# AI4Science-WestlakeU/wdno

Hardware: AMD Instinct MI355X
Metric: diffusion train steps/sec, 2D smoke U-Net (8 samples per GPU per step) (higher is better)
Workload: dtype f32

## Files before the change

### include/wdno_hip.h

```cpp
#ifndef WDNO_HIP_H
#define WDNO_HIP_H
#include <stdint.h>
#include <stddef.h>

#ifdef __cplusplus
extern "C" {
#endif

typedef void* wdno_stream_t;

enum { WDNO_OK = 0, WDNO_EINVAL = -1, WDNO_ELAUNCH = -2, WDNO_EUNSUPPORTED = -3, WDNO_EWORKSPACE = -4 };

#define WDNO_AMAX_SLOTS 64
#define WDNO_AMAX_STRIDE 16
#define WDNO_AMAX_FLOATS (WDNO_AMAX_SLOTS * WDNO_AMAX_STRIDE)
const char* wdno_strerror(int code);
int wdno_version(void);
const char* wdno_last_hip_error(void);
int wdno_set_debug(int mode);

typedef struct {
  int nd;
  int mode;
  int L;
  int n_img;
  int in_dims[3];
  int out_dims[3];
  int64_t cs_img, cs_band, cs0, cs1;
} wdno_dwt_desc;
size_t wdno_dwt_ws_bytes(const wdno_dwt_desc* d);
int wdno_dwt_fwd(const float* x, float* coef, const wdno_dwt_desc* d, const float* filters_host, void* ws, size_t ws_bytes, wdno_stream_t s);
int wdno_dwt_inv(const float* coef, float* x, const wdno_dwt_desc* d, const float* filters_host, void* ws, size_t ws_bytes, wdno_stream_t s);
int wdno_dwt_fwd_adjoint(const float* dcoef, float* dx, const wdno_dwt_desc* d, const float* filters_host, void* ws, size_t ws_bytes, wdno_stream_t s);
int wdno_dwt_inv_adjoint(const float* dx, float* dcoef, const wdno_dwt_desc* d, const float* filters_host, void* ws, size_t ws_bytes, wdno_stream_t s);
int wdno_dwt_fwd_packed(const float* x, float* state, const wdno_dwt_desc* d, const float* filters_host, int img_inner, int64_t cs_outer, int row_w,
                        const float* rescaler, wdno_stream_t s);
int wdno_upsample_coef(const float* in, float* out, int64_t outer, int a, int mid, int b, int c, int fa, int fb, int fc, wdno_stream_t s);
int wdno_pack_smoke_state(const float* coef, int64_t coef_sim_stride, const float* init_coef, int64_t init_sim_stride, const float* smokeout,
                          int64_t so_sim_stride, const int64_t* idx, const float* rescaler, float* state, int64_t B, int F, int nt, int nx,
                          int pad_t, int pad_x, wdno_stream_t s);
int wdno_pack_smoke_fields(const float* coef, int64_t coef_sim_stride, const float* rho0, int64_t rho0_sim_stride, const float* curve,
                           int64_t curve_sim_stride, const float* dec_lo_host, const float* dec_hi_host, int L, const float* rescaler,
                           float* state, int64_t B, int F, int nt, int nx, int pad_t, int pad_x, int H0, int W0, int T0, wdno_stream_t s);

int wdno_nc_to_cl(const float* src, float* dst, int64_t N, int C, int64_t S, int Cp, wdno_stream_t s);
int wdno_cl_to_nc(const float* src, float* dst, int64_t N, int C, int64_t S, int Cp, wdno_stream_t s);
int wdno_concat2_cl_planes(const float* a, int Ca, const float* b, int Cb, const float* rec_a, const float* rec_b, void* hi, void* lo,
                           float* scale_out, int64_t P, wdno_stream_t s);
int wdno_concat2_cl(const float* a, int Ca, const float* b, int Cb, float* out, int64_t P, wdno_stream_t s);
int wdno_concat2_cl_amax(const float* a, int Ca, const float* b, int Cb, float* out, float* amax_rec, int64_t P, wdno_stream_t s);
int wdno_split2_cl(const float* in, float* a, int Ca, float* b, int Cb, int64_t P, wdno_stream_t s);
int wdno_upsample2x_cl_fwd(const float* in, float* out, int64_t N, int H, int W, int C, wdno_stream_t s);
int wdno_upsample2x_cl_bwd(const float* dout, float* din, int64_t N, int H, int W, int C, wdno_stream_t s);

typedef struct {
  int N, D, H, W, C;
  int OD, OH, OW, K;
  int kd, kh, kw;
  int sd, sh, sw;
  int pd, ph, pw;
  int YD, YH, YW;
  int osd, osh, osw, ood, ooh, oow;
} wdno_conv_geom;
int wdno_conv_fwd(const float* x, const float* wp, const float* bias, const float* residual, float* y,
                  const wdno_conv_geom* g, wdno_stream_t s);
int wdno_amax(const float* x, int64_t n, float* amax_zeroed, wdno_stream_t s);
int wdno_amax_record(const float* x, int64_t n, float* rec_zeroed, wdno_stream_t s);
int wdno_split_f16(const float* x, const float* amax_rec, void* hi, void* lo, float* scale_out, int64_t rows, int C, int C8, wdno_stream_t s);
size_t wdno_split_colsum_ws_bytes(int64_t rows, int C8);
int wdno_split_f16_colsum(const float* x, const float* amax_rec, void* hi, void* lo, float* scale_out, float* colsum_out,
                          void* ws, size_t ws_bytes, int64_t rows, int C, int C8, wdno_stream_t s);
int wdno_pack_split_weight(const float* w, const float* amax, void* hi, void* lo, float* scale_out, int K, int C, int kd, int kh, int kw,
                           int A, int B, int mode, wdno_stream_t s);
typedef struct { const void* x; int64_t n; void* out; } wdno_amax_item;
typedef struct {
  const void* w; const void* amax; void* hi; void* lo; void* scale_out;
  int K, C, kd, kh, kw, A, B, mode;
} wdno_wsplit_item;
int wdno_amax_multi(const void* table, int n_items, int blocks_per_item, wdno_stream_t s);
int wdno_pack_split_weight_multi(const void* table, int n_items, int blocks_per_item, wdno_stream_t s);
int wdno_conv_fwd_f16x3(const void* xh, const void* xl, const float* sx, const void* wph, const void* wpl, const float* sw,
                        const float* bias, const float* residual, float* y, const wdno_conv_geom* g, wdno_stream_t s);
int wdno_conv_fwd_f16x3_amax(const void* xh, const void* xl, const float* sx, const void* wph, const void* wpl, const float* sw,
                             const float* bias, const float* residual, float* y, float* amax_rec, const wdno_conv_geom* g,
                             wdno_stream_t s);
typedef struct { int channels, d0, h0, w0; } wdno_zero_box;
int wdno_conv_fwd_f16x3_zbox(const void* xh, const void* xl, const float* sx, const void* wph, const void* wpl, const float* sw,
                             const float* bias, const float* residual, float* y, float* amax_rec, const wdno_conv_geom* g,
                             const wdno_zero_box* zb, wdno_stream_t s);
int wdno_conv_fwd_bf16_ex(const void* x16, const void* wp16, const float* bias, const float* residual, void* y, int y_bf16, float* amax_rec,
                          const wdno_conv_geom* g, const wdno_zero_box* zb, wdno_stream_t s);
int wdno_conv_fwd_f16x3_ws(const void* xh, const void* xl, const float* sx, const void* wph, const void* wpl, const float* sw,
                           const float* bias, const float* residual, float* y, float* amax_rec, const wdno_conv_geom* g,
                           void* ws, size_t ws_bytes, wdno_stream_t s);
size_t wdno_conv_fwd_split_ws_bytes(const wdno_conv_geom* g);
size_t wdno_conv_wgrad_f16x3_ws_bytes(const wdno_conv_geom* g);
int wdno_conv_pixel_table(void* table, const wdno_conv_geom* g, wdno_stream_t s);
int wdno_conv_wgrad_f16x3(const void* xh, const void* xl, const float* sx, const void* dyh, const void* dyl, const float* sdy,
                          const void* pixel_table, float* dwp, void* ws, size_t ws_bytes, const wdno_conv_geom* g, wdno_stream_t s);
int wdno_conv_wgrad_f16x3_param(const void* xh, const void* xl, const float* sx, const void* dyh, const void* dyl, const float* sdy,
                                const void* pixel_table, float* dw, int Kn, int Cn, void* ws, size_t ws_bytes,
                                const wdno_conv_geom* g, wdno_stream_t s);
#define WDNO_WGRAD_REDUCE_MAX 40
typedef struct wdno_wgrad_reduce_item {
  const float* ws; float* dw;
  int n, splits;
  int K8, C8, kw, ntap, Kn, Cn;
  int tiled;
  int reserved;
} wdno_wgrad_reduce_item;
int wdno_conv_wgrad_partials(const void* xh, const void* xl, const float* sx, const void* dyh, const void* dyl, const float* sdy,
                             const void* pixel_table, float* dw, int Kn, int Cn, void* ws, size_t ws_bytes,
                             const wdno_conv_geom* g, wdno_wgrad_reduce_item* item, wdno_stream_t s);
int wdno_wgrad_reduce_multi(const wdno_wgrad_reduce_item* items, int n_items, wdno_stream_t s);
size_t wdno_conv_wgrad_ws_bytes(const wdno_conv_geom* g);
int wdno_conv_wgrad(const float* x, const float* dy, float* dwp, void* ws, size_t ws_bytes,
                    const wdno_conv_geom* g, wdno_stream_t s);
#define WDNO_ROWS_SUM_MAX 64
typedef struct wdno_rows_sum_item {
  const void* part; float* out;
  int rows, stride, col0, ncols;
  int is_double, reserved;
} wdno_rows_sum_item;
int wdno_rows_sum_multi(const wdno_rows_sum_item* items, int n_items, wdno_stream_t s);
size_t wdno_colsum_ws_bytes(int64_t P, int C);
int wdno_colsum(const float* in, float* out, int64_t P, int C, void* ws, size_t ws_bytes, wdno_stream_t s);

int wdno_cast_bf16(const float* x, void* out16, int64_t rows, int C, int C8, wdno_stream_t s);
int wdno_cast_bf16_colsum(const float* x, void* out16, float* colsum_out, void* ws, size_t ws_bytes, int64_t rows, int C, int C8, wdno_stream_t s);
int wdno_conv_fwd_bf16(const void* x16, const void* wp16, const float* bias, const float* residual, float* y, float* amax_rec,
                       const wdno_conv_geom* g, wdno_stream_t s);
int wdno_conv_wgrad_bf16_param(const void* x16, const void* dy16, const void* pixel_table, float* dw, int Kn, int Cn, void* ws,
                               size_t ws_bytes, const wdno_conv_geom* g, wdno_stream_t s);

size_t wdno_groupnorm_ws_bytes(int64_t N, int64_t S, int C, int G);
size_t wdno_groupnorm_stats_floats(int64_t N, int C, int G);
int wdno_groupnorm_act_fwd(const float* x, const float* gamma, const float* beta, const float* ss, float* y,
                           float* stats, int64_t N, int64_t S, int C, int G, float eps, int silu,
                           void* ws, size_t ws_bytes, wdno_stream_t s);
int wdno_groupnorm_act_fwd_amax(const float* x, const float* gamma, const float* beta, const float* ss, float* y,
                                float* stats, float* amax_rec, int64_t N, int64_t S, int C, int G, float eps, int silu,
                                void* ws, size_t ws_bytes, wdno_stream_t s);
int wdno_groupnorm_act_bwd(const float* x, const float* dy, const float* gamma, const float* beta, const float* ss,
                           const float* stats, float* dx, float* dgb_partial, float* dss,
                           int64_t N, int64_t S, int C, int G, int silu, void* ws, size_t ws_bytes, wdno_stream_t s);
int wdno_groupnorm_act_bwd_amax(const float* x, const float* dy, const float* gamma, const float* beta, const float* ss,
                                const float* stats, float* dx, float* dgb_partial, float* dss, float* amax_rec,
                                int64_t N, int64_t S, int C, int G, int silu, void* ws, size_t ws_bytes, wdno_stream_t s);
size_t wdno_groupnorm_bwd_planes_ws_bytes(int64_t N, int64_t S, int C, int G);
size_t wdno_groupnorm_fwd_planes_ws_bytes(int64_t N, int64_t S, int C, int G);
int wdno_groupnorm_act_fwd_planes(const float* x, const float* gamma, const float* beta, const float* ss, void* y_hi, void* y_lo,
                                  float* y_scale, float* stats, float* bound_rec, int64_t N, int64_t S, int C, int G, float eps, int silu,
                                  void* ws, size_t ws_bytes, wdno_stream_t s);
int wdno_groupnorm_act_add_fwd_planes(const float* x, const float* gamma, const float* beta, const float* ss, const float* residual,
                                      const float* res_rec, float* y, void* y_hi, void* y_lo, float* y_scale, float* stats,
                                      float* bound_rec, float* y_amax_rec, int64_t N, int64_t S, int C, int G, float eps, int silu,
                                      void* ws, size_t ws_bytes, wdno_stream_t s);
int wdno_groupnorm_act_bwd_planes(const float* x, const float* dy, const float* gamma, const float* beta, const float* ss,
                                  const float* stats, void* dx_hi, void* dx_lo, float* dx_scale, float* dx_colsum,
                                  float* dgb_partial, float* dgb_sum, float* dss, float* bound_rec, int64_t N, int64_t S, int C, int G, int silu,
                                  void* ws, size_t ws_bytes, wdno_stream_t s);
int wdno_groupnorm_bwd_planes_tail(int64_t N, int64_t S, int C, int G, size_t* csp_offset, int* rows);
int wdno_groupnorm_act_fwd_amax_t(const void* x, int x_bf16, const float* gamma, const float* beta, const float* ss, float* y,
// ... 224 lines not shown
```

### wdno_amd/_lib.py

```python
import contextlib
import ctypes as C
import os

import torch

HERE = os.path.dirname(os.path.abspath(__file__))
LIB_PATH = os.path.join(HERE, 'libwdno_hip.so')

P = C.c_void_p
I = C.c_int
L = C.c_int64
F = C.c_float
Z = C.c_size_t


class DwtDesc(C.Structure):
    _fields_ = [('nd', I), ('mode', I), ('L', I), ('n_img', I), ('in_dims', I * 3), ('out_dims', I * 3),
                ('cs_img', L), ('cs_band', L), ('cs0', L), ('cs1', L)]


class ConvGeom(C.Structure):
    _fields_ = [(k, I) for k in ('N', 'D', 'H', 'W', 'C', 'OD', 'OH', 'OW', 'K', 'kd', 'kh', 'kw', 'sd', 'sh', 'sw',
                                 'pd', 'ph', 'pw', 'YD', 'YH', 'YW', 'osd', 'osh', 'osw', 'ood', 'ooh', 'oow')]


class AttnDesc(C.Structure):
    _fields_ = [('n_uo', I), ('n_ui', I), ('n_tok', I), ('heads', I), ('so', L), ('si', L), ('st', L)]


class CondDesc(C.Structure):
    _fields_ = [(k, I) for k in ('tree', 'B', 'F', 'C', 'H', 'W', 'cT', 'cH', 'cW', 'cond_pad', 'cond_a', 'cond_b',
                                 'cond_c', 'cond_low', 'u_rows', 'uT_rows')]


class WgradReduceItem(C.Structure):
    _fields_ = [('ws', C.c_void_p), ('dw', C.c_void_p), ('n', I), ('splits', I), ('K8', I), ('C8', I), ('kw', I), ('ntap', I), ('Kn', I), ('Cn', I),
                ('tiled', I), ('reserved', I)]


class RowsSumItem(C.Structure):
    _fields_ = [('part', C.c_void_p), ('out', C.c_void_p), ('rows', I), ('stride', I), ('col0', I), ('ncols', I), ('is_double', I), ('reserved', I)]


class BurgersDesc(C.Structure):
    _fields_ = [(k, I) for k in ('N', 's', 'nx0', 'nt_f', 'nxf', 'steps', 'record_time', 'f_time', 'num_t', 'sub_s', 'out_cols', 'waves',
                                 'points')] + [(k, F) for k in ('c', 'd', 'dm', 'dt')]


class BurgersGenerateDesc(C.Structure):
    _fields_ = [(k, I) for k in ('N', 's', 't', 'steps', 'record_time', 'f_time', 'num_t', 'st', 'sx', 'f_rows', 'cols', 'waves', 'points',
                                 'clamp')] + [(k, F) for k in ('c', 'd', 'dm', 'dt', 'alpha')]


class BurgersGuidanceDesc(C.Structure):
    _fields_ = [(k, I) for k in ('B', 'C', 'H', 'W', 'sample_stride', 'chan_stride', 'row_stride', 'h', 'w', 'n_t', 'n_x', 'L', 'mode', 'ntile',
                                 'tw', 'lds_bytes', 'num_timesteps', 'condition_f', 'clip_x0')] + [(k, F) for k in ('wu', 'wf')]


class SmokeGuidanceDesc(C.Structure):
    _fields_ = [(k, I) for k in ('B', 'F', 'C', 'H', 'W', 'sample_stride', 'frame_stride', 'chan_stride', 'row_stride', 'tc', 'hc', 'wc', 'to', 'ho',
                                 'wo', 'L', 'mode', 'half', 'num_timesteps', 'clip_x0', 'is_condition_control', 'has_init_u', 'tn', 'hn', 'kt', 'kh',
                                 'ncopy', 'lds1_bytes', 'lds2_bytes')] + [(k, F) for k in ('w_energy', 'w_init')]


class SmokeSolveDesc(C.Structure):
    _fields_ = [(k, I) for k in ('B', 'nt', 'nx', 'time_interval', 'space_interval', 'num_t', 'max_iter', 'n_out', 'threads')] + [('accuracy', F)]


class SmokeGenerateDesc(C.Structure):
    _fields_ = [(k, I) for k in ('B', 'scenelength', 'record_scale', 'stride', 'max_iter', 'threads', 'noise_mode')] + [('accuracy', F), ('seed', C.c_uint64)]


PD, PG, PA, PC = C.POINTER(DwtDesc), C.POINTER(ConvGeom), C.POINTER(AttnDesc), C.POINTER(CondDesc)
PF = C.POINTER(C.c_float)

PROTOTYPES = {
    'wdno_strerror': (C.c_char_p, [I]),
    'wdno_version': (I, []),
    'wdno_last_hip_error': (C.c_char_p, []),
    'wdno_set_debug': (I, [I]),
    'wdno_dwt_ws_bytes': (Z, [PD]),
    'wdno_dwt_fwd': (I, [P, P, PD, PF, P, Z, P]),
    'wdno_dwt_fwd_packed': (I, [P, P, PD, PF, I, L, I, P, P]),
    'wdno_dwt_inv': (I, [P, P, PD, PF, P, Z, P]),
    'wdno_dwt_fwd_adjoint': (I, [P, P, PD, PF, P, Z, P]),
    'wdno_dwt_inv_adjoint': (I, [P, P, PD, PF, P, Z, P]),
    'wdno_upsample_coef': (I, [P, P, L, I, I, I, I, I, I, I, P]),
    'wdno_pack_smoke_state': (I, [P, L, P, L, P, L, P, P, P, L, I, I, I, I, I, P]),
    'wdno_pack_smoke_fields': (I, [P, L, P, L, P, L, PF, PF, I, P, P, L, I, I, I, I, I, I, I, I, P]),
    'wdno_nc_to_cl': (I, [P, P, L, I, L, I, P]),
    'wdno_cl_to_nc': (I, [P, P, L, I, L, I, P]),
    'wdno_concat2_cl': (I, [P, I, P, I, P, L, P]),
    'wdno_concat2_cl_planes': (I, [P, I, P, I, P, P, P, P, P, L, P]),
    'wdno_concat2_cl_amax': (I, [P, I, P, I, P, P, L, P]),
    'wdno_split2_cl': (I, [P, P, I, P, I, L, P]),
    'wdno_upsample2x_cl_fwd': (I, [P, P, L, I, I, I, P]),
    'wdno_upsample2x_cl_bwd': (I, [P, P, L, I, I, I, P]),
    'wdno_conv_fwd': (I, [P, P, P, P, P, PG, P]),
    'wdno_amax': (I, [P, L, P, P]),
    'wdno_amax_record': (I, [P, L, P, P]),
    'wdno_split_f16': (I, [P, P, P, P, P, L, I, I, P]),
    'wdno_split_colsum_ws_bytes': (Z, [L, I]),
    'wdno_split_f16_colsum': (I, [P, P, P, P, P, P, P, Z, L, I, I, P]),
    'wdno_pack_split_weight': (I, [P, P, P, P, P, I, I, I, I, I, I, I, I, P]),
    'wdno_amax_multi': (I, [P, I, I, P]),
    'wdno_pack_split_weight_multi': (I, [P, I, I, P]),
    'wdno_conv_fwd_f16x3': (I, [P, P, P, P, P, P, P, P, P, PG, P]),
    'wdno_conv_fwd_f16x3_amax': (I, [P, P, P, P, P, P, P, P, P, P, PG, P]),
    'wdno_conv_fwd_f16x3_ws': (I, [P, P, P, P, P, P, P, P, P, P, PG, P, Z, P]),
    'wdno_conv_fwd_split_ws_bytes': (Z, [PG]),
    'wdno_conv_wgrad_f16x3_ws_bytes': (Z, [PG]),
    'wdno_conv_pixel_table': (I, [P, PG, P]),
    'wdno_conv_wgrad_f16x3': (I, [P, P, P, P, P, P, P, P, P, Z, PG, P]),
    'wdno_conv_wgrad_f16x3_param': (I, [P, P, P, P, P, P, P, P, I, I, P, Z, PG, P]),
    'wdno_conv_wgrad_partials': (I, [P, P, P, P, P, P, P, P, I, I, P, Z, PG, P, P]),
    'wdno_wgrad_reduce_multi': (I, [P, I, P]),
    'wdno_rows_sum_multi': (I, [P, I, P]),
    'wdno_cast_bf16': (I, [P, P, L, I, I, P]),
    'wdno_cast_bf16_colsum': (I, [P, P, P, P, Z, L, I, I, P]),
    'wdno_conv_fwd_bf16': (I, [P, P, P, P, P, P, PG, P]),
    'wdno_conv_fwd_f16x3_zbox': (I, [P, P, P, P, P, P, P, P, P, P, PG, P, P]),
    'wdno_conv_fwd_bf16_ex': (I, [P, P, P, P, P, I, P, PG, P, P]),
    'wdno_conv_wgrad_bf16_param': (I, [P, P, P, P, I, I, P, Z, PG, P]),
    'wdno_conv_wgrad_ws_bytes': (Z, [PG]),
    'wdno_conv_wgrad': (I, [P, P, P, P, Z, PG, P]),
    'wdno_colsum_ws_bytes': (Z, [L, I]),
    'wdno_colsum': (I, [P, P, L, I, P, Z, P]),
    'wdno_groupnorm_ws_bytes': (Z, [L, L, I, I]),
    'wdno_groupnorm_stats_floats': (Z, [L, I, I]),
    'wdno_groupnorm_act_fwd': (I, [P, P, P, P, P, P, L, L, I, I, F, I, P, Z, P]),
    'wdno_groupnorm_act_fwd_amax': (I, [P, P, P, P, P, P, P, L, L, I, I, F, I, P, Z, P]),
    'wdno_groupnorm_act_bwd': (I, [P, P, P, P, P, P, P, P, P, L, L, I, I, I, P, Z, P]),
    'wdno_groupnorm_act_bwd_amax': (I, [P, P, P, P, P, P, P, P, P, P, L, L, I, I, I, P, Z, P]),
    'wdno_groupnorm_bwd_planes_ws_bytes': (Z, [L, L, I, I]),
    'wdno_groupnorm_bwd_planes_tail': (I, [L, L, I, I, C.POINTER(Z), C.POINTER(I)]),
    'wdno_groupnorm_fwd_planes_ws_bytes': (Z, [L, L, I, I]),
    'wdno_groupnorm_act_fwd_planes': (I, [P, P, P, P, P, P, P, P, P, L, L, I, I, F, I, P, Z, P]),
    'wdno_groupnorm_act_add_fwd_planes': (I, [P, P, P, P, P, P, P, P, P, P, P, P, P, L, L, I, I, F, I, P, Z, P]),
    'wdno_layernorm_fwd_planes': (I, [P, P, P, P, P, L, I, F, P]),
    'wdno_groupnorm_act_bwd_planes': (I, [P, P, P, P, P, P, P, P, P, P, P, P, P, P, L, L, I, I, I, P, Z, P]),
    'wdno_groupnorm_act_fwd_amax_t': (I, [P, I, P, P, P, P, P, P, L, L, I, I, F, I, P, Z, P]),
    'wdno_groupnorm_act_fwd_planes_t': (I, [P, I, P, P, P, P, P, P, P, P, L, L, I, I, F, I, P, Z, P]),
    'wdno_groupnorm_act_add_fwd_planes_t': (I, [P, I, P, P, P, P, P, P, P, P, P, P, P, P, L, L, I, I, F, I, P, Z, P]),
    'wdno_groupnorm_act_bwd_planes_t': (I, [P, I, P, I, P, P, P, P, P, P, P, P, P, P, P, P, L, L, I, I, I, P, Z, P]),
    'wdno_layernorm_fwd': (I, [P, P, P, L, I, F, P]),
    'wdno_layernorm_fwd_amax': (I, [P, P, P, P, L, I, F, P]),
    'wdno_layernorm_bwd_ws_bytes': (Z, [L, I]),
    'wdno_layernorm_bwd': (I, [P, P, P, P, P, L, I, F, P, Z, P]),
    'wdno_layernorm_bwd_add': (I, [P, P, P, P, P, P, L, I, F, P, Z, P]),
    'wdno_layernorm_bwd_add_amax': (I, [P, P, P, P, P, P, P, L, I, F, P, Z, P]),
    'wdno_attn_fwd': (I, [P, P, P, P, P, PA, F, P]),
    'wdno_attn_bwd_ws_bytes': (Z, [PA]),
    'wdno_attn_bwd': (I, [P, P, P, P, P, P, P, P, PA, F, P, Z, P]),
    'wdno_attn_fwd_amax': (I, [P, P, P, P, P, P, PA, F, P]),
    'wdno_attn_bwd_amax': (I, [P, P, P, P, P, P, P, P, P, PA, F, P, Z, P]),
    'wdno_attn_fwd_planes': (I, [P, P, P, P, P, P, P, P, P, P, PA, F, P]),
    'wdno_linattn_fwd_planes': (I, [P, P, P, P, P, P, P, L, I, I, F, P]),
    'wdno_attn_bwd_planes': (I, [P, P, P, P, P, P, P, P, P, P, P, P, PA, F, P, Z, P]),
    'wdno_tattn_fused_takes': (I, [I, I, I]),
    'wdno_tattn_fused_fwd': (I, [P, P, F, P, P, P, P, P, P, P, P, P, P, P, P, P, L, I, L, I, I, F, P]),
    'wdno_lattn_fused_takes': (I, [I, I, I]),
    'wdno_lattn_fused_ws_bytes': (Z, [L, I]),
    'wdno_lattn_fused_fwd': (I, [P, P, F, P, P, P, P, P, P, P, P, P, P, P, P, Z, L, I, I, I, F, P]),
    'wdno_lattn_fused_bwd_grads': (I, []),
    'wdno_lattn_fused_bwd_ws_bytes': (Z, [L, I]),
    'wdno_lattn_fused_bwd': (I, [P, P, P, F, P, P, P, P, P, P, P, P, P, P, P, P, P, Z, L, I, I, I, F, P]),
    'wdno_tattn_fused_bwd_ws_bytes': (Z, []),
    'wdno_tattn_fused_bwd_grads': (I, []),
    'wdno_tattn_fused_bwd': (I, [P, P, P, F, P, P, P, P, P, P, P, P, P, P, P, P, P, P, P, Z, L, I, L, I, I, F, P]),
    'wdno_linattn_ws_bytes': (Z, [L, I]),
    'wdno_linattn_fwd': (I, [P, P, P, P, L, I, I, F, P]),
    'wdno_linattn_bwd': (I, [P, P, P, P, P, P, Z, L, I, I, F, P]),
    'wdno_linattn_fwd_amax': (I, [P, P, P, P, P, L, I, I, F, P]),
    'wdno_linattn_bwd_amax': (I, [P, P, P, P, P, P, P, Z, L, I, I, F, P]),
    'wdno_linattn_bwd_planes': (I, [P, P, P, P, P, P, P, P, P, P, P, Z, L, I, I, F, P]),
    'wdno_act_fwd': (I, [P, P, L, I, P]),
    'wdno_act_bwd': (I, [P, P, P, L, I, P]),
    'wdno_linear_rows_fwd': (I, [P, I, P, I, P, P, I, I, I, I, P]),
    'wdno_linear_rows_wgrad': (I, [P, I, P, I, P, P, I, I, I, P]),
    'wdno_linear_multi_fwd': (I, [P, I, I, P, P, I, I, P]),
    'wdno_linear_multi_wgrad': (I, [P, I, I, P, P, P, P, I, I, P]),
    'wdno_linear_multi_dgrad_ws_bytes': (Z, [I, I, I]),
    'wdno_linear_multi_dgrad': (I, [P, I, I, P, P, I, I, P, Z, P]),
    'wdno_add': (I, [P, P, P, L, P]),
    'wdno_add_amax': (I, [P, P, P, P, L, P]),
    'wdno_sinusoidal_emb': (I, [P, P, P, I, I, P]),
    'wdno_q_sample_cond': (I, [P, P, P, P, P, P, P, PC, P]),
    'wdno_apply_cond': (I, [P, P, PC, P]),
    'wdno_weighted_mse_ws_bytes': (Z, [L]),
# ... 64 lines not shown
```

### wdno_amd/csrc/conv_h3.hip

```cpp
#include "conv_common.h"
#include <type_traits>
#include <algorithm>

typedef _Float16 half8 __attribute__((ext_vector_type(8)));
typedef __bf16 bf16x8 __attribute__((ext_vector_type(8)));
template <bool LP>
__device__ __forceinline__ f32x16 mfma_16(half8 a, half8 b, f32x16 c) {
  if constexpr (LP) return __builtin_amdgcn_mfma_f32_32x32x16_bf16(__builtin_bit_cast(bf16x8, a), __builtin_bit_cast(bf16x8, b), c, 0, 0, 0);
  else return __builtin_amdgcn_mfma_f32_32x32x16_f16(a, b, c, 0, 0, 0);
}

#define HBK 32
#define HST 40

template <bool RECORD>
__global__ __launch_bounds__(256) void amax_kernel(const float* __restrict__ x, int64_t n, unsigned* __restrict__ out) {
  __shared__ float red[4];
  const int64_t n4 = n >> 2;
  const float4* x4 = reinterpret_cast<const float4*>(x);
  float m = 0.f;
  const int64_t stride = (int64_t)gridDim.x * 1024;
  for (int64_t k0 = (int64_t)blockIdx.x * 1024 + threadIdx.x; k0 < n4; k0 += stride) {
    float4 v[4];
#pragma unroll
// ... 1135 lines not shown
      const int dz = ps_div(tap, khw, m_khw), rr = tap - dz * khw;
      const int dy = ps_div(rr, kw, m_kw), dx = rr - dy * kw;
      const int ts = mode ? T - 1 - tap : tap;
      const int a = (mode ? c0 : k0) + al;
      const int bg = ((mode ? k0 : c0) >> 3) + g;
      if (a >= A || bg >= b8) continue;
      const float* src = mode ? tile + (ts * pt.KT + g * 8) * pt.CTp + al : tile + (ts * pt.KT + al) * pt.CTp + g * 8;
      const int step = mode ? pt.CTp : 1;
      half8 h, l;
      typedef unsigned short us8 __attribute__((ext_vector_type(8)));
      us8 bq;
#pragma unroll
      for (int e = 0; e < 8; ++e) {
        const float v = src[e * step];
        const float tv = v * s;
        const _Float16 th = (_Float16)tv;
        h[e] = th;
        l[e] = (_Float16)(tv - (float)th);
        bq[e] = bf16_rne(v);
      }
      int64_t i = ((((int64_t)dz * kh + dy) * A + a) * kw + dx) * b8 + bg;
      if (frag) {
        const int li = a & 31, t = bg >> 2, hh2 = (bg >> 1) & 1, s2 = bg & 1;
        if (frag == 1) { const int ti = a >> 7, hd = (a >> 5) & 3; i = ((((hd * 3 + ti) * (B >> 5) + t) * 2 + s2) * 64 + hh2 * 32 + li); }
        else { const int q4 = A >> 2, wv = a / q4, mt = (a - wv * q4) >> 5; i = ((((wv * (A >> 7) + mt) * 4 + t) * 2 + s2) * 64 + hh2 * 32 + li); }
      }
      if (lp) { *reinterpret_cast<us8*>(hi + i * 8) = bq; continue; }
      *reinterpret_cast<half8*>(hi + i * 8) = h;
      *reinterpret_cast<half8*>(lo + i * 8) = l;
    }
  }
}
__global__ __launch_bounds__(256) void pack_split_weight_kernel(const float* __restrict__ w, const float* __restrict__ amax,
                                                                 _Float16* __restrict__ hi, _Float16* __restrict__ lo,
                                                                 float* __restrict__ scale_out, int K, int C, int kd, int kh, int kw,
                                                                 int A, int B, int mode) {
  pack_split_body(w, amax, hi, lo, scale_out, K, C, kd, kh, kw, A, B, mode, (int)blockIdx.x, (int)gridDim.x);
}
__global__ __launch_bounds__(256) void amax_multi_kernel(const wdno_amax_item* __restrict__ tab) {
  __shared__ float red[4];
  const wdno_amax_item it = tab[blockIdx.y];
  const float* x = (const float*)it.x;
  const int64_t n = it.n;
  float m = 0.f;
  int64_t head = (int64_t)(((16 - (reinterpret_cast<uintptr_t>(x) & 15)) & 15) >> 2);
  if (head > n) head = n;
  const int64_t n4 = (n - head) >> 2, tail0 = head + 4 * n4;
  if (blockIdx.x == 0) {
    if ((int64_t)threadIdx.x < head) m = fabsf(x[threadIdx.x]);
    if (tail0 + (int64_t)threadIdx.x < n) m = fmaxf(m, fabsf(x[tail0 + threadIdx.x]));
  }
  const float4* x4 = reinterpret_cast<const float4*>(x + head);
  const int64_t stride = (int64_t)gridDim.x * 256;
  int64_t k = (int64_t)blockIdx.x * 256 + threadIdx.x;
  for (; k + 3 * stride < n4; k += 4 * stride) {
    const float4 a = x4[k], b = x4[k + stride], c = x4[k + 2 * stride], d = x4[k + 3 * stride];
    m = amax4(amax4(m, a), b);
    m = amax4(amax4(m, c), d);
  }
  for (; k < n4; k += stride) m = amax4(m, x4[k]);
  m = wave_max(m);
  if ((threadIdx.x & 63) == 0) red[threadIdx.x >> 6] = m;
  __syncthreads();
  if (threadIdx.x == 0) {
    m = fmaxf(fmaxf(red[0], red[1]), fmaxf(red[2], red[3]));
    if (m > 0.f) atomicMax((unsigned*)it.out, __float_as_uint(m));
  }
}
extern "C" int wdno_amax_multi(const void* table, int n_items, int blocks_per_item, wdno_stream_t s) {
  WDNO_REQUIRE(table && n_items > 0 && n_items <= 65535 && blocks_per_item > 0);
  amax_multi_kernel<<<dim3((unsigned)blocks_per_item, (unsigned)n_items), 256, 0, as_stream(s)>>>((const wdno_amax_item*)table);
  return wdno_check_launch();
}
__global__ __launch_bounds__(256) void pack_split_weight_multi_kernel(const wdno_wsplit_item* __restrict__ tab) {
  const wdno_wsplit_item it = tab[blockIdx.y];
  pack_split_body((const float*)it.w, (const float*)it.amax, (_Float16*)it.hi, (_Float16*)it.lo, (float*)it.scale_out, it.K, it.C, it.kd, it.kh,
                  it.kw, it.A, it.B, it.mode, (int)blockIdx.x, (int)gridDim.x);
}
extern "C" int wdno_pack_split_weight_multi(const void* table, int n_items, int blocks_per_item, wdno_stream_t s) {
  WDNO_REQUIRE(table && n_items > 0 && n_items <= 65535 && blocks_per_item > 0);
  pack_split_weight_multi_kernel<<<dim3((unsigned)blocks_per_item, (unsigned)n_items), 256, 0, as_stream(s)>>>((const wdno_wsplit_item*)table);
  return wdno_check_launch();
}
extern "C" int wdno_pack_split_weight(const float* w, const float* amax, void* hi, void* lo, float* scale_out, int K, int C, int kd, int kh,
                                      int kw, int A, int B, int mode, wdno_stream_t s) {
  WDNO_REQUIRE(K > 0 && C > 0 && kd > 0 && kh > 0 && kw > 0 && A > 0 && B > 0 && (B & 7) == 0 && mode >= 0 && mode <= 11);
  WDNO_REQUIRE(mode < 2 || mode > 5 || (kd == 1 && kh == 2 && kw == 2));
  WDNO_REQUIRE(mode < 6 || (kd == 1 && kh == 1 && kw == 1));
  WDNO_REQUIRE(mode != 1 && (mode < 6 || mode >= 10) ? (A >= K && B >= C) : (A >= C && B >= K));
  WDNO_REQUIRE(mode != 10 || (A == 384 && (B & 31) == 0 && lo != nullptr));
  WDNO_REQUIRE(mode != 11 || (B == 128 && (A & 127) == 0 && lo != nullptr));
  WDNO_REQUIRE(lo == nullptr || (amax != nullptr && scale_out != nullptr));
  int64_t total = (int64_t)kd * kh * A * kw * (B / 8);
  const PackTile ptile = pack_tile(kd * kh * kw, A, B, mode == 1 || (mode >= 6 && mode < 10) ? 1 : 0);
  if ((int64_t)kd * kh * kw * ptile.KT * ptile.CTp > PS_LDS_FLOATS + 16) return WDNO_EUNSUPPORTED;
  (void)total;
  pack_split_weight_kernel<<<std::min(2048, ptile.tiles_k * ptile.tiles_c), 256, 0, as_stream(s)>>>(w, amax, (_Float16*)hi, (_Float16*)lo, scale_out, K, C, kd, kh, kw,
                                                                            A, B, mode);
  return wdno_check_launch();
}
```

### wdno_amd/ops.py

```python
import contextlib
import ctypes as C
import math
import os

import torch

from . import _lib
from ._lib import AttnDesc, CondDesc, ConvGeom, DwtDesc

WEIGHT_EPOCH = 0
_pack_cache = {}


PROFILE = None


class _timed:

    def __init__(self, key, flops):
        self.key, self.flops = key, flops

    def __enter__(self):
        if PROFILE is not None:
            self.e0 = torch.cuda.Event(enable_timing=True)
# ... 422 lines not shown


def split_f16(x2d, amax=None, c8=None):
    rows, c = x2d.shape
    if c8 is None or _lp():
        c8 = pad8(c)
    lib = _lib_()
    if _lp():
        hi = torch.empty((rows, c8), device=x2d.device, dtype=torch.float16)
        _lib.check(lib.wdno_cast_bf16(_p(x2d), _p(hi), rows, c, c8, _stream()), 'cast_bf16')
        return hi, None, None
    if amax is None:
        amax = tensor_amax(x2d)
    hi = torch.empty((rows, c8), device=x2d.device, dtype=torch.float16)
    lo = torch.empty((rows, c8), device=x2d.device, dtype=torch.float16)
    scale = amax[1:2]
    _lib.check(lib.wdno_split_f16(_p(x2d), _p(amax), _p(hi), _p(lo), _p(scale), rows, c, c8, _stream()), 'split_f16')
    return hi, lo, scale


def split_f16_colsum(x2d, amax=None, bias=None, k=None):
    rows, c = x2d.shape
    c8 = pad8(c)
    g8 = c8 // 8
    if g8 > 256 or (g8 & (g8 - 1)):
        return split_f16(x2d, amax), colsum(x2d)
    lib = _lib_()
    nb = lib.wdno_split_colsum_ws_bytes(rows, c8)
    ws = _ws(nb, x2d.device)
    flat = None
    if bias is not None and DEFER_ROW_SUMS and _WGRAD_PENDING is not None:
        flat = _flat_grad_out(bias, (k,))
    cs = None if flat is not None else torch.empty(c8, device=x2d.device, dtype=torch.float32)
    if _lp():
        hi = torch.empty((rows, c8), device=x2d.device, dtype=torch.float16)
        _lib.check(lib.wdno_cast_bf16_colsum(_p(x2d), _p(hi), _p(cs), _p(ws), nb, rows, c, c8, _stream()), 'cast_bf16_colsum')
        planes = (hi, None, None)
    else:
        if amax is None:
            amax = tensor_amax(x2d)
        hi = torch.empty((rows, c8), device=x2d.device, dtype=torch.float16)
        lo = torch.empty((rows, c8), device=x2d.device, dtype=torch.float16)
        scale = amax[1:2]
        _lib.check(lib.wdno_split_f16_colsum(_p(x2d), _p(amax), _p(hi), _p(lo), _p(scale), _p(cs), _p(ws), nb, rows, c, c8, _stream()), 'split_f16_colsum')
        planes = (hi, lo, scale)
    if flat is not None:
        return planes, rows_sum_for_param(_RowsJob(ws, ws.data_ptr(), nb // (8 * c8), c8, 0, k, 1), bias, out=flat)
    return planes, cs[:c]


class _WPlan:
    __slots__ = ('w', 'wd', 'kind', 'cp8', 'kp', 'hi', 'lo', 'sc', 'ver', 'used', 'lp')


def _wmode(kind):
    if kind[0] == 'q':
        return 6 + 2 * int(kind[1]) + int(kind[2])
    if kind[0] == 'a':
        return 10 if kind == 'aq' else 11
    return 0 if kind == 'f' else 1 if kind == 'd' else 2 + 2 * int(kind[1]) + int(kind[2])


def _wdims(kind, w5):
    if kind[0] == 'p':
        assert tuple(w5.shape[2:]) == (1, 4, 4)
        return w5.shape[1], w5.shape[0], 1, 2, 2
    if kind[0] == 'q':
        assert tuple(w5.shape[2:]) == (1, 2, 2)
        return w5.shape[0], w5.shape[1], 1, 1, 1
    return tuple(w5.shape)


_wplans = {}
_wtables = {}


class _AmaxItem(C.Structure):
    _fields_ = [('x', C.c_void_p), ('n', C.c_int64), ('out', C.c_void_p)]


class _WsplitItem(C.Structure):
    _fields_ = [('w', C.c_void_p), ('amax', C.c_void_p), ('hi', C.c_void_p), ('lo', C.c_void_p), ('scale_out', C.c_void_p),
                ('K', C.c_int), ('C', C.c_int), ('kd', C.c_int), ('kh', C.c_int), ('kw', C.c_int), ('A', C.c_int), ('B', C.c_int), ('mode', C.c_int)]


def _refresh_weight_plans(epoch_used, lp=None):
    if lp is None:
        lp = _lp()
    keys = tuple(k for k, pl in _wplans.items() if pl.used >= epoch_used - 3 and pl.wd.is_contiguous() and pl.lp == lp)
    if len(keys) < 2:
        return
    dev = _wplans[keys[0]].wd.device
    tabs = _wtables.get(keys)
    if tabs is None:
        while len(_wtables) >= 8:
            _wtables.pop(next(iter(_wtables)))
        wptrs = []
        for k in keys:
            pl = _wplans[k]
            if pl.wd.data_ptr() not in wptrs:
                wptrs.append(pl.wd.data_ptr())
        amax = torch.zeros(len(wptrs), device=dev, dtype=torch.float32)
        seen = {}
        aitems = (_AmaxItem * len(wptrs))()
        for k in keys:
            pl = _wplans[k]
            i = wptrs.index(pl.wd.data_ptr())
            if i not in seen:
                seen[i] = True
                aitems[i] = _AmaxItem(pl.wd.data_ptr(), pl.wd.numel(), amax.data_ptr() + 4 * i)
        sitems = (_WsplitItem * len(keys))()
        for j, k in enumerate(keys):
            pl = _wplans[k]
            kk, cc, kd, kh, kw = _wdims(pl.kind, _as5(pl.wd))
            i = wptrs.index(pl.wd.data_ptr())
            if lp:
                sitems[j] = _WsplitItem(pl.wd.data_ptr(), None, pl.hi.data_ptr(), None, None, kk, cc, kd, kh, kw, pl.kp, pl.cp8, _wmode(pl.kind))
                continue
            sitems[j] = _WsplitItem(pl.wd.data_ptr(), amax.data_ptr() + 4 * i, pl.hi.data_ptr(), pl.lo.data_ptr(), pl.sc.data_ptr(),
                                    kk, cc, kd, kh, kw, pl.kp, pl.cp8, _wmode(pl.kind))
        at = torch.frombuffer(bytearray(bytes(aitems)), dtype=torch.uint8).to(dev)
        stt = torch.frombuffer(bytearray(bytes(sitems)), dtype=torch.uint8).to(dev)
        tabs = (amax, at, stt, len(wptrs))
        _wtables[keys] = tabs
    amax, at, stt, nw = tabs
    lib = _lib_()
    with torch.no_grad():
        if not lp:
            amax.zero_()
            _lib.check(lib.wdno_amax_multi(_p(at), nw, 64, _stream()), 'amax_multi')
        _lib.check(lib.wdno_pack_split_weight_multi(_p(stt), len(keys), 256, _stream()), 'pack_split_weight_multi')
    for k in keys:
        pl = _wplans[k]
        pl.ver = (pl.w._version, WEIGHT_EPOCH)


def cache_snapshot():
    return [dict(_pack_cache), dict(_wplans), dict(_wtables), dict(_lin_tables), dict(_rot_cache), dict(_pixel_tables), dict(_freq_cache),
            {k: v[0] for k, v in _amax_pool.items()}]


def captured_plans(since=None):
    return [pl for pl in _wplans.values() if since is None or pl.used >= since]


def touch_plans(plans):
    e = WEIGHT_EPOCH
    for pl in plans:
        pl.used = e


def prepare_graph_refresh():
    epoch = WEIGHT_EPOCH
    for pl in _wplans.values():
        if pl.used >= epoch - 3:
            pl.used = epoch
    bump_weight_epoch(params=False)
    if _wplans:
        for lp in {pl.lp for pl in _wplans.values()}:
            _refresh_weight_plans(WEIGHT_EPOCH, lp)
    bump_weight_epoch(params=False)


def split_weight(w, kind, cp8, kp, pack=None):
    lp = _lp()
    key = (w.data_ptr(), kind, cp8, kp, tuple(w.shape), tuple(w.stride()), lp)
    ver = (w._version, WEIGHT_EPOCH)
    pl = _wplans.get(key)
    if pl is not None:
        if pl.ver != ver:
            _refresh_weight_plans(WEIGHT_EPOCH)
        if pl.ver == ver:
            pl.used = WEIGHT_EPOCH
            return pl.hi, pl.lo, pl.sc
    with torch.no_grad():
        wd = w.detach()
        wc = wd if wd.is_contiguous() else wd.contiguous()
        amax = None
        if not lp:
            amax = torch.zeros(1, device=w.device, dtype=torch.float32)
            _lib.check(_lib_().wdno_amax(_p(wc), wc.numel(), _p(amax), _stream()), 'amax')
        k, c, kd, kh, kw = _wdims(kind, _as5(wc))
        rows = kd * kh * kp * kw
        if pl is None:
            pl = _WPlan()
            pl.w, pl.wd, pl.kind, pl.cp8, pl.kp, pl.lp = wd, wd, kind, cp8, kp, lp
            pl.hi = torch.empty((rows, cp8), device=w.device, dtype=torch.float16)
            pl.lo = None if lp else torch.empty((rows, cp8), device=w.device, dtype=torch.float16)
            pl.sc = None if lp else torch.empty(1, device=w.device, dtype=torch.float32)
            if len(_wplans) > 4096:
                _wplans.clear(); _wtables.clear()
                bump_weight_epoch(params=False)
                ver = (w._version, WEIGHT_EPOCH)
            _wplans[key] = pl
        _lib.check(_lib_().wdno_pack_split_weight(_p(wc), _p(amax), _p(pl.hi), _p(pl.lo), _p(pl.sc), k, c, kd, kh, kw, kp, cp8,
                                                  _wmode(kind), _stream()), 'pack_split_weight')
    pl.ver = ver
    pl.used = WEIGHT_EPOCH
    return pl.hi, pl.lo, pl.sc


ACT16 = os.environ.get('WDNO_ACT16', '0') == '1'
ZERO_BOX = True


class _ZeroBox(C.Structure):
    _fields_ = [('channels', C.c_int), ('d0', C.c_int), ('h0', C.c_int), ('w0', C.c_int)]


def set_zero_box(t, box):
    t._wdno_zero_box = (tuple(int(v) for v in box), t._version)
    return t


# ... 1375 lines not shown
```

Baseline: 33.15.

## Pack paired weight layouts from one LDS tile in a persistent kernel

```diff
diff --git a/include/wdno_hip.h b/include/wdno_hip.h
--- a/include/wdno_hip.h
+++ b/include/wdno_hip.h
@@ -79,6 +79,14 @@
 } wdno_wsplit_item;
 int wdno_amax_multi(const void* table, int n_items, int blocks_per_item, wdno_stream_t s);
 int wdno_pack_split_weight_multi(const void* table, int n_items, int blocks_per_item, wdno_stream_t s);
+typedef struct { void* hi; void* lo; void* scale_out; int A, B, mode, reserved; } wdno_wsplit_out;
+typedef struct {
+  const void* w; const void* amax;
+  int K, C, kd, kh, kw, n_out, KT, CT;
+  wdno_wsplit_out out[2];
+} wdno_wsplit_pair_item;
+int wdno_wsplit_pair_tiles(wdno_wsplit_pair_item* item);
+int wdno_pack_split_weight_paired(const void* table, const void* first, int n_items, int total_tiles, wdno_stream_t s);
 int wdno_conv_fwd_f16x3(const void* xh, const void* xl, const float* sx, const void* wph, const void* wpl, const float* sw,
                         const float* bias, const float* residual, float* y, const wdno_conv_geom* g, wdno_stream_t s);
 int wdno_conv_fwd_f16x3_amax(const void* xh, const void* xl, const float* sx, const void* wph, const void* wpl, const float* sw,
diff --git a/wdno_amd/_lib.py b/wdno_amd/_lib.py
--- a/wdno_amd/_lib.py
+++ b/wdno_amd/_lib.py
@@ -105,6 +105,8 @@
     'wdno_pack_split_weight': (I, [P, P, P, P, P, I, I, I, I, I, I, I, I, P]),
     'wdno_amax_multi': (I, [P, I, I, P]),
     'wdno_pack_split_weight_multi': (I, [P, I, I, P]),
+    'wdno_wsplit_pair_tiles': (I, [P]),
+    'wdno_pack_split_weight_paired': (I, [P, P, I, I, P]),
     'wdno_conv_fwd_f16x3': (I, [P, P, P, P, P, P, P, P, P, PG, P]),
     'wdno_conv_fwd_f16x3_amax': (I, [P, P, P, P, P, P, P, P, P, P, PG, P]),
     'wdno_conv_fwd_f16x3_ws': (I, [P, P, P, P, P, P, P, P, P, P, PG, P, Z, P]),
diff --git a/wdno_amd/csrc/conv_h3.hip b/wdno_amd/csrc/conv_h3.hip
--- a/wdno_amd/csrc/conv_h3.hip
+++ b/wdno_amd/csrc/conv_h3.hip
@@ -1241,6 +1241,220 @@
   pack_split_weight_multi_kernel<<<dim3((unsigned)blocks_per_item, (unsigned)n_items), 256, 0, as_stream(s)>>>((const wdno_wsplit_item*)table);
   return wdno_check_launch();
 }
+#define PSP_THREADS 512
+#define PSP_LDS_FLOATS 20480
+__host__ __device__ static inline int psp_class(int mode) { return mode == 1 || (mode >= 6 && mode < 10) ? 1 : 0; }
+static inline bool psp_choose_tile(wdno_wsplit_pair_item* it) {
+  const int T = it->kd * it->kh * it->kw;
+  auto fits = [&](int kt, int ct) { return (int64_t)T * kt * (ct + 1) <= PSP_LDS_FLOATS; };
+  int kt, ct;
+  if (it->n_out == 1) {
+    int longd = 128, shortd = 8;
+    const int cls = psp_class(it->out[0].mode);
+    auto f1 = [&]() { return cls ? fits(longd, shortd) : fits(shortd, longd); };
+    while (longd > 8 && !f1()) longd >>= 1;
+    while (shortd > 1 && !f1()) shortd >>= 1;
+    if (!f1()) return false;
+    kt = cls ? longd : shortd; ct = cls ? shortd : longd;
+  } else {
+    kt = 64; ct = 64;
+    while (kt >= 8 && !fits(kt, ct)) {
+      if (kt == ct) kt >>= 1; else ct >>= 1;
+    }
+    if (kt < 8) return false;
+  }
+  it->KT = kt; it->CT = ct;
+  return true;
+}
+__host__ __device__ static inline PackTile psp_tile(const wdno_wsplit_pair_item& it) {
+  PackTile t;
+  t.KT = it.KT; t.CT = it.CT; t.CTp = it.CT + 1;
+  int kext = 0, cext = 0;
+#pragma unroll
+  for (int o = 0; o < 2; ++o) {
+    if (o >= it.n_out) break;
+    const int cls = psp_class(it.out[o].mode);
+    kext = max(kext, cls ? it.out[o].B : it.out[o].A);
+    cext = max(cext, cls ? it.out[o].A : it.out[o].B);
+  }
+  t.tiles_k = (kext + t.KT - 1) / t.KT;
+  t.tiles_c = (cext + t.CT - 1) / t.CT;
+  return t;
+}
+__global__ __launch_bounds__(PSP_THREADS) void pack_split_weight_paired_kernel(const wdno_wsplit_pair_item* __restrict__ tab,
+                                                                                const int* __restrict__ first, int n_items, int total) {
+  extern __shared__ float tile[];
+  for (int t = blockIdx.x; t < total; t += gridDim.x) {
+    int ilo = 0, ihi = n_items - 1;
+    while (ilo < ihi) {
+      const int mid = (ilo + ihi + 1) >> 1;
+      if (first[mid] <= t) ilo = mid; else ihi = mid - 1;
+    }
+    const wdno_wsplit_pair_item it = tab[ilo];
+    const int tl = t - first[ilo];
+    const float* __restrict__ w = (const float*)it.w;
+    const int K = it.K, C = it.C, kh = it.kh, kw = it.kw;
+    const int T = it.kd * kh * kw, khw = kh * kw;
+    const int mode0 = it.out[0].mode;
+    const int parity = mode0 >= 2 && mode0 < 6 ? mode0 - 2 : -1;
+    const int patch = mode0 >= 6 && mode0 < 10 ? mode0 - 6 : -1;
+    const PackTile pt = psp_tile(it);
+    if (pt.KT <= 0 || (int64_t)T * pt.KT * pt.CTp > PSP_LDS_FLOATS) continue;
+    const int tk = tl / pt.tiles_c, tc = tl - tk * pt.tiles_c;
+    const int k0 = tk * pt.KT, c0 = tc * pt.CT;
+    const int run = pt.CT * T;
+    const int cvalid = min(pt.CT, C - c0);
+    const unsigned m_T = ps_magic(T);
+    __syncthreads();
+    if (parity < 0 && patch < 0) {
+      const int S = (run + 6) >> 2;
+      const unsigned m_S = ps_magic(S);
+      const int64_t row0 = ((int64_t)k0 * C + c0) * T;
+      const int phase0 = (int)((reinterpret_cast<uintptr_t>(w + row0) >> 2) & 3), dphase = (int)(((int64_t)C * T) & 3);
+      const int nslot = pt.KT * S;
+      for (int idx0 = threadIdx.x; idx0 < nslot; idx0 += PSP_THREADS * 4) {
+        float4 v[4];
+        int kks[4], e0s[4];
+#pragma unroll
+        for (int u = 0; u < 4; ++u) {
+          const int idx = idx0 + PSP_THREADS * u;
+          const bool active = idx < nslot;
+          const int kk = active ? ps_div(idx, S, m_S) : 0, j = idx - kk * S;
+          const int len = active && k0 + kk < K && cvalid > 0 ? cvalid * T : 0;
+          const int e0 = 4 * j - ((phase0 + kk * dphase) & 3);
+          const float* row = w + row0 + (int64_t)kk * C * T;
+          const bool full = e0 >= 0 && e0 + 4 <= len;
+          v[u] = *reinterpret_cast<const float4*>(full ? (const void*)(row + e0) : (const void*)tab);
+          kks[u] = active ? kk : -1; e0s[u] = e0;
+          if (!full) {
+            v[u] = make_float4(0.f, 0.f, 0.f, 0.f);
+            if (e0 + 0 >= 0 && e0 + 0 < len) v[u].x = row[e0 + 0];
+            if (e0 + 1 >= 0 && e0 + 1 < len) v[u].y = row[e0 + 1];
+            if (e0 + 2 >= 0 && e0 + 2 < len) v[u].z = row[e0 + 2];
+            if (e0 + 3 >= 0 && e0 + 3 < len) v[u].w = row[e0 + 3];
+          }
+        }
+#pragma unroll
+        for (int u = 0; u < 4; ++u) {
+          if (kks[u] < 0) continue;
+          const float vv[4] = {v[u].x, v[u].y, v[u].z, v[u].w};
+#pragma unroll
+          for (int q = 0; q < 4; ++q) {
+            const int e = e0s[u] + q;
+            if (e < 0 || e >= run) continue;
+            const int cl = ps_div(e, T, m_T), tap = e - cl * T;
+            tile[(tap * pt.KT + kks[u]) * pt.CTp + cl] = vv[q];
+          }
+        }
+      }
+    } else {
+      const unsigned m_run = ps_magic(run);
+      const int nload = pt.KT * run;
+      for (int idx0 = threadIdx.x; idx0 < nload; idx0 += PSP_THREADS * 8) {
+        float v[8];
+        int dst[8];
+#pragma unroll
+        for (int u = 0; u < 8; ++u) {
+          const int idx = min(idx0 + PSP_THREADS * u, nload - 1);
+          const int kk = ps_div(idx, run, m_run), r = idx - kk * run;
+          const int cl = ps_div(r, T, m_T), tap = r - cl * T;
+          const bool ok = k0 + kk < K && cl < cvalid;
+          const int64_t off = !ok ? 0 : patch >= 0 ? (((int64_t)(k0 + kk) * C + c0 + cl) * 4 + patch)
+                              : ((int64_t)(c0 + cl) * K + (k0 + kk)) * 16 + (3 - (parity >> 1) - 2 * (tap >> 1)) * 4 + (3 - (parity & 1) - 2 * (tap & 1));
+          v[u] = w[off];
+          if (!ok) v[u] = 0.f;
+          dst[u] = idx0 + PSP_THREADS * u < nload ? (tap * pt.KT + kk) * pt.CTp + cl : -1;
+        }
+#pragma unroll
+        for (int u = 0; u < 8; ++u)
+          if (dst[u] >= 0) tile[dst[u]] = v[u];
+      }
+    }
+    __syncthreads();
+#pragma unroll
+    for (int o = 0; o < 2; ++o) {
+      if (o >= it.n_out) break;
+      const wdno_wsplit_out out = it.out[o];
+      _Float16* __restrict__ hi = (_Float16*)out.hi;
+      _Float16* __restrict__ lo = (_Float16*)out.lo;
+      const int A = out.A, b8 = out.B >> 3;
+      const int frag = out.mode >= 10 ? out.mode - 9 : 0;
+      const int mode = psp_class(out.mode);
+      const bool lp = lo == nullptr;
+      const float s = lp ? 1.0f : scale_from_amax(((const float*)it.amax)[0]);
+      if (!lp && tl == 0 && threadIdx.x == 0) ((float*)out.scale_out)[0] = s;
+      const int bt8 = (mode ? pt.KT : pt.CT) >> 3;
+      const int at = mode ? pt.CT : pt.KT;
+      const unsigned m_bt8 = ps_magic(bt8), m_at = ps_magic(at), m_khw = ps_magic(khw), m_kw = ps_magic(kw);
+      const int nitems = T * at * bt8;
+      for (int idx = threadIdx.x; idx < nitems; idx += PSP_THREADS) {
+        int q = ps_div(idx, bt8, m_bt8);
+        const int g = idx - q * bt8;
+        const int tap = ps_div(q, at, m_at), al = q - tap * at;
+        const int dz = ps_div(tap, khw, m_khw), rr = tap - dz * khw;
+        const int dy = ps_div(rr, kw, m_kw), dx = rr - dy * kw;
+        const int ts = mode ? T - 1 - tap : tap;
+        const int a = (mode ? c0 : k0) + al;
+        const int bg = ((mode ? k0 : c0) >> 3) + g;
+        if (a >= A || bg >= b8) continue;
+        const float* src = mode ? tile + (ts * pt.KT + g * 8) * pt.CTp + al : tile + (ts * pt.KT + al) * pt.CTp + g * 8;
+        const int step = mode ? pt.CTp : 1;
+        half8 h, l;
+        typedef unsigned short us8 __attribute__((ext_vector_type(8)));
+        us8 bq;
+#pragma unroll
+        for (int e = 0; e < 8; ++e) {
+          const float v = src[e * step];
+          const float tv = v * s;
+          const _Float16 th = (_Float16)tv;
+          h[e] = th;
+          l[e] = (_Float16)(tv - (float)th);
+          bq[e] = bf16_rne(v);
+        }
+        int64_t i = ((((int64_t)dz * kh + dy) * A + a) * kw + dx) * b8 + bg;
+        if (frag) {
+          const int B = out.B;
+          const int li = a & 31, t2 = bg >> 2, hh2 = (bg >> 1) & 1, s2 = bg & 1;
+          if (frag == 1) { const int ti = a >> 7, hd = (a >> 5) & 3; i = ((((hd * 3 + ti) * (B >> 5) + t2) * 2 + s2) * 64 + hh2 * 32 + li); }
+          else { const int q4 = A >> 2, wv = a / q4, mt = (a - wv * q4) >> 5; i = ((((wv * (A >> 7) + mt) * 4 + t2) * 2 + s2) * 64 + hh2 * 32 + li); }
+        }
+        if (lp) { *reinterpret_cast<us8*>(hi + i * 8) = bq; continue; }
+        *reinterpret_cast<half8*>(hi + i * 8) = h;
+        *reinterpret_cast<half8*>(lo + i * 8) = l;
+      }
+    }
+  }
+}
+static bool psp_out_ok(const wdno_wsplit_pair_item& it, const wdno_wsplit_out& o) {
+  const int mode = o.mode, K = it.K, C = it.C, A = o.A, B = o.B;
+  if (!(A > 0 && B > 0 && (B & 7) == 0 && mode >= 0 && mode <= 11 && o.hi)) return false;
+  if (mode >= 2 && mode <= 5 && !(it.kd == 1 && it.kh == 2 && it.kw == 2)) return false;
+  if (mode >= 6 && !(it.kd == 1 && it.kh == 1 && it.kw == 1)) return false;
+  if (!(mode != 1 && (mode < 6 || mode >= 10) ? (A >= K && B >= C) : (A >= C && B >= K))) return false;
+  if (mode == 10 && !(A == 384 && (B & 31) == 0 && o.lo)) return false;
+  if (mode == 11 && !(B == 128 && (A & 127) == 0 && o.lo)) return false;
+  return o.lo == nullptr || (it.amax != nullptr && o.scale_out != nullptr);
+}
+extern "C" int wdno_wsplit_pair_tiles(wdno_wsplit_pair_item* it) {
+  WDNO_REQUIRE(it && it->w && it->K > 0 && it->C > 0 && it->kd > 0 && it->kh > 0 && it->kw > 0 && (it->n_out == 1 || it->n_out == 2));
+  for (int o = 0; o < it->n_out; ++o) WDNO_REQUIRE(psp_out_ok(*it, it->out[o]));
+  if (it->n_out == 2) {
+    WDNO_REQUIRE(it->out[0].mode <= 1 && it->out[1].mode <= 1);
+    WDNO_REQUIRE((it->out[0].lo == nullptr) == (it->out[1].lo == nullptr));
+  }
+  if (!psp_choose_tile(it)) return it->n_out == 2 ? 0 : WDNO_EUNSUPPORTED;
+  const PackTile pt = psp_tile(*it);
+  const int64_t tiles = (int64_t)pt.tiles_k * pt.tiles_c;
+  return tiles > 0 && tiles < (1 << 24) ? (int)tiles : WDNO_EUNSUPPORTED;
+}
+extern "C" int wdno_pack_split_weight_paired(const void* table, const void* first, int n_items, int total_tiles, wdno_stream_t s) {
+  WDNO_REQUIRE(table && first && n_items > 0 && total_tiles >= n_items);
+  const int grid = std::min(total_tiles, 2 * std::max(1, wdno_num_cus()));
+  static const hipError_t attr = hipFuncSetAttribute((const void*)pack_split_weight_paired_kernel, hipFuncAttributeMaxDynamicSharedMemorySize, PSP_LDS_FLOATS * 4);
+  if (attr != hipSuccess) return WDNO_ELAUNCH;
+  pack_split_weight_paired_kernel<<<grid, PSP_THREADS, PSP_LDS_FLOATS * 4, as_stream(s)>>>((const wdno_wsplit_pair_item*)table, (const int*)first, n_items, total_tiles);
+  return wdno_check_launch();
+}
 extern "C" int wdno_pack_split_weight(const float* w, const float* amax, void* hi, void* lo, float* scale_out, int K, int C, int kd, int kh,
                                       int kw, int A, int B, int mode, wdno_stream_t s) {
   WDNO_REQUIRE(K > 0 && C > 0 && kd > 0 && kh > 0 && kw > 0 && A > 0 && B > 0 && (B & 7) == 0 && mode >= 0 && mode <= 11);
diff --git a/wdno_amd/ops.py b/wdno_amd/ops.py
--- a/wdno_amd/ops.py
+++ b/wdno_amd/ops.py
@@ -528,6 +528,60 @@
 class _WsplitItem(C.Structure):
     _fields_ = [('w', C.c_void_p), ('amax', C.c_void_p), ('hi', C.c_void_p), ('lo', C.c_void_p), ('scale_out', C.c_void_p),
                 ('K', C.c_int), ('C', C.c_int), ('kd', C.c_int), ('kh', C.c_int), ('kw', C.c_int), ('A', C.c_int), ('B', C.c_int), ('mode', C.c_int)]
+
+
+class _WsplitOut(C.Structure):
+    _fields_ = [('hi', C.c_void_p), ('lo', C.c_void_p), ('scale_out', C.c_void_p), ('A', C.c_int), ('B', C.c_int), ('mode', C.c_int), ('reserved', C.c_int)]
+
+
+class _WsplitPairItem(C.Structure):
+    _fields_ = [('w', C.c_void_p), ('amax', C.c_void_p), ('K', C.c_int), ('C', C.c_int), ('kd', C.c_int), ('kh', C.c_int), ('kw', C.c_int),
+                ('n_out', C.c_int), ('KT', C.c_int), ('CT', C.c_int), ('out', _WsplitOut * 2)]
+
+
+PAIRED_WEIGHT_REFRESH = True
+
+
+def _paired_tables(sitems, dev):
+    lib = _lib_()
+
+    def out_of(it):
+        return _WsplitOut(it.hi, it.lo, it.scale_out, it.A, it.B, it.mode, 0)
+
+    def item_of(its):
+        a = its[0]
+        pit = _WsplitPairItem(a.w, a.amax, a.K, a.C, a.kd, a.kh, a.kw, len(its), 0, 0)
+        for o, it in enumerate(its):
+            pit.out[o] = out_of(it)
+        return pit
+
+    groups = {}
+    for j, it in enumerate(sitems):
+        key = (it.w, it.K, it.C, it.kd, it.kh, it.kw) if it.mode <= 1 else (j,)
+        groups.setdefault(key, []).append(it)
+    pitems, first = [], [0]
+    for its in groups.values():
+        while its:
+            pit, n = None, 0
+            if len(its) >= 2 and its[0].mode != its[1].mode:
+                pit = item_of(its[:2])
+                n = lib.wdno_wsplit_pair_tiles(C.byref(pit))
+            if n > 0:
+                its = its[2:]
+            else:
+                pit = item_of(its[:1])
+                n = lib.wdno_wsplit_pair_tiles(C.byref(pit))
+                its = its[1:]
+            if n <= 0:
+                raise RuntimeError(f'wdno_wsplit_pair_tiles: {n}')
+            pitems.append(pit)
+            first.append(first[-1] + n)
+    if first[-1] >= 2 ** 31:
+        raise RuntimeError('weight refresh: tile count overflows')
+    arr = (_WsplitPairItem * len(pitems))(*pitems)
+    ptt = torch.frombuffer(bytearray(bytes(arr)), dtype=torch.uint8).to(dev)
+    pfirst = torch.tensor(first, dtype=torch.int32).to(dev)
+    return ptt, pfirst, len(pitems), first[-1]
 
 
 def _refresh_weight_plans(epoch_used, lp=None):
@@ -567,15 +621,18 @@
                                     kk, cc, kd, kh, kw, pl.kp, pl.cp8, _wmode(pl.kind))
         at = torch.frombuffer(bytearray(bytes(aitems)), dtype=torch.uint8).to(dev)
         stt = torch.frombuffer(bytearray(bytes(sitems)), dtype=torch.uint8).to(dev)
-        tabs = (amax, at, stt, len(wptrs))
+        tabs = (amax, at, stt, len(wptrs)) + _paired_tables(sitems, dev)
         _wtables[keys] = tabs
-    amax, at, stt, nw = tabs
+    amax, at, stt, nw, ptt, pfirst, npair, ntiles = tabs
     lib = _lib_()
     with torch.no_grad():
         if not lp:
             amax.zero_()
             _lib.check(lib.wdno_amax_multi(_p(at), nw, 64, _stream()), 'amax_multi')
-        _lib.check(lib.wdno_pack_split_weight_multi(_p(stt), len(keys), 256, _stream()), 'pack_split_weight_multi')
+        if PAIRED_WEIGHT_REFRESH:
+            _lib.check(lib.wdno_pack_split_weight_paired(_p(ptt), _p(pfirst), npair, ntiles, _stream()), 'pack_split_weight_paired')
+        else:
+            _lib.check(lib.wdno_pack_split_weight_multi(_p(stt), len(keys), 256, _stream()), 'pack_split_weight_multi')
     for k in keys:
         pl = _wplans[k]
         pl.ver = (pl.w._version, WEIGHT_EPOCH)
```

After: 33.15. About the same (-0.0%).
